# GuixingLin/akka-allreduce

Hardware: AMD Instinct MI355X
Metric: allreduce algbw (GB/s) on 256 MB fp32 buffer at 1/2/4/8 MI355X (higher is better)
Workload: dtype fp32

## Files before the change

### akka_allreduce_amd/models/mlp.py

```python
from __future__ import annotations

from typing import Optional

import torch
import torch.nn as nn
import torch.nn.functional as F

from ..ops.colsum import colsum
from ..ops.xent import cross_entropy
from ..parallel.dp import AllreduceFn, GradientBucket


def _mm_into(a: torch.Tensor, b: torch.Tensor, out: torch.Tensor) -> None:
    if a.dtype == out.dtype:
        torch.mm(a, b, out=out)
        return
    try:
        torch.mm(a, b, out_dtype=out.dtype, out=out)
    except (TypeError, RuntimeError):
        out.copy_(torch.mm(a, b))


class _LinearIntoBucket(torch.autograd.Function):

    @staticmethod
    def forward(ctx, x, w, b, gw, gb, ws=None, bs=None):
        dt = torch.get_autocast_dtype(x.device.type) if torch.is_autocast_enabled(x.device.type) else None
        with torch.autocast(device_type=x.device.type, enabled=False):
            if dt is not None and ws is not None and bs is not None and ws.dtype == dt and bs.dtype == dt:
                xc, wc, bc = x.to(dt), ws, bs
            elif dt is not None:
                xc, wc, bc = x.to(dt), w.to(dt), b.to(dt)
            else:
                xc, wc, bc = x, w, b
            y = F.linear(xc, wc, bc)
        ctx.save_for_backward(xc, wc)
        ctx.gw, ctx.gb = gw, gb
        return y

    @staticmethod
    def backward(ctx, go):
        xc, wc = ctx.saved_tensors
        go2 = go.reshape(-1, go.shape[-1]).to(wc.dtype)
        _mm_into(go2.t(), xc.reshape(-1, xc.shape[-1]), ctx.gw)
        if go2.is_cuda and go2.dtype == torch.bfloat16 and ctx.gb.dtype == torch.float32 and ctx.gb.is_contiguous():
            colsum(go2, out=ctx.gb.view(-1))
        else:
            torch.sum(go2, 0, dtype=ctx.gb.dtype, out=ctx.gb)
        gx = (go2 @ wc).reshape(*go.shape[:-1], wc.shape[1]) if ctx.needs_input_grad[0] else None
        return gx, None, None, None, None, None, None


class _LinearReluIntoBucket(torch.autograd.Function):

    @staticmethod
    def forward(ctx, x, w, b, gw, gb, ws, bs):
        dt = torch.get_autocast_dtype(x.device.type)
        with torch.autocast(device_type=x.device.type, enabled=False):
            xc = x.to(dt)
            wc = ws if ws is not None else w.to(dt)
            bc = bs if bs is not None else b.to(dt)
            x2 = xc.reshape(-1, xc.shape[-1])
            h = torch._addmm_activation(bc, x2, wc.t(), use_gelu=False)
        ctx.save_for_backward(x2, wc, h)
        ctx.gw, ctx.gb, ctx.xshape = gw, gb, xc.shape
        return h.reshape(*xc.shape[:-1], wc.shape[0])

    @staticmethod
    def backward(ctx, go):
        x2, wc, h = ctx.saved_tensors
        go2 = go.reshape(-1, go.shape[-1]).to(wc.dtype).contiguous()
        g = torch.empty_like(go2)
        colsum(go2, out=ctx.gb.view(-1), relu_of=h, masked_out=g)
        _mm_into(g.t(), x2, ctx.gw)
        gx = (g @ wc).reshape(ctx.xshape) if ctx.needs_input_grad[0] else None
        return gx, None, None, None, None, None, None


class MLP(nn.Module):
    def __init__(self, d_in: int, d_hidden: int, d_out: int):
        super().__init__()
        self.fc1 = nn.Linear(d_in, d_hidden)
        self.fc2 = nn.Linear(d_hidden, d_out)
        self.direct_grads = False
        self.last_step_direct = False
        self.shadow_bucket: Optional[GradientBucket] = None

    def _linear(self, fc: nn.Linear, x: torch.Tensor) -> torch.Tensor:
        if self.direct_grads and torch.is_grad_enabled():
            sb = self.shadow_bucket
            ws = sb.shadow_of(fc.weight) if sb is not None else None
            bs = sb.shadow_of(fc.bias) if sb is not None else None
            return _LinearIntoBucket.apply(x, fc.weight, fc.bias, fc.weight.grad, fc.bias.grad, ws, bs)
        return fc(x)

    def _linear_relu(self, fc: nn.Linear, x: torch.Tensor) -> torch.Tensor:
        if (self.direct_grads and torch.is_grad_enabled() and x.is_cuda and torch.is_autocast_enabled("cuda")
                and torch.get_autocast_dtype("cuda") == torch.bfloat16 and fc.bias is not None
                and fc.bias.grad is not None and fc.bias.grad.is_contiguous()):
            sb = self.shadow_bucket
            ws = sb.shadow_of(fc.weight) if sb is not None else None
            bs = sb.shadow_of(fc.bias) if sb is not None else None
            return _LinearReluIntoBucket.apply(x, fc.weight, fc.bias, fc.weight.grad, fc.bias.grad, ws, bs)
        return F.relu(self._linear(fc, x))

    def forward(self, x: torch.Tensor) -> torch.Tensor:
        return self._linear(self.fc2, self._linear_relu(self.fc1, x))


def dp_sgd_step(model: nn.Module, x: torch.Tensor, y: torch.Tensor, lr: float,
                allreduce: Optional[AllreduceFn], bucket: Optional[GradientBucket] = None,
                sync_loss: bool = True, compute_dtype: Optional[torch.dtype] = None,
                direct_grads: bool = True, shadow_weights: bool = True, fused_loss: bool = True,
                optimizer=None):
    if optimizer is not None:
        if bucket is not None and optimizer.bucket is not bucket:
            raise ValueError("dp_sgd_step: the optimizer was built on another bucket")
        bucket = optimizer.bucket
    if bucket is None:
        bucket = getattr(model, "_akka_bucket", None)
        if bucket is None:
            bucket = GradientBucket(list(model.parameters()))
            model._akka_bucket = bucket
    loss = _forward_backward(model, x, y, bucket, compute_dtype, direct_grads, shadow_weights, fused_loss)
    bucket.update_from(allreduce, lr, optimizer or bucket.sgd)
    return float(loss.detach()) if sync_loss else loss.detach()


def _forward_backward(model: nn.Module, x: torch.Tensor, y: torch.Tensor, bucket: GradientBucket,
                      compute_dtype: Optional[torch.dtype], direct_grads: bool, shadow_weights: bool,
                      fused_loss: bool, grad_seed: Optional[torch.Tensor] = None) -> torch.Tensor:
    bucket.rebind()
    direct = isinstance(model, MLP) and direct_grads and bucket.bound() \
        and set(map(id, model.parameters())) == set(map(id, bucket.params))
    try:
        if direct:
            model.direct_grads = True
            lowp = compute_dtype if (shadow_weights and compute_dtype is not None
                                     and compute_dtype != torch.float32) else None
            model.shadow_bucket = bucket if bucket.use_shadow(lowp) else None
        else:
            bucket.use_shadow(None)
            bucket.zero_()
        if compute_dtype is not None and compute_dtype != torch.float32:
            with torch.autocast(device_type=x.device.type, dtype=compute_dtype):
                logits = model(x)
            loss = cross_entropy(logits, y) if fused_loss else F.cross_entropy(logits.float(), y)
        else:
            loss = F.cross_entropy(model(x), y)
        loss.backward(grad_seed)
    finally:
        if isinstance(model, MLP):
            model.direct_grads = False
            model.shadow_bucket = None
            model.last_step_direct = direct
    return loss


class GraphedDPStep:

    def __init__(self, model: "MLP", bucket: GradientBucket, x: torch.Tensor, y: torch.Tensor,
                 compute_dtype: Optional[torch.dtype] = None, shadow_weights: bool = True, warmup: int = 3,
                 allreduce: Optional[AllreduceFn] = None, lr: Optional[float] = None, optimizer=None):
        if not (x.is_cuda and isinstance(model, MLP)):
            raise ValueError("GraphedDPStep: an MLP on a GPU")
        if optimizer is not None and optimizer.bucket is not bucket:
            raise ValueError("GraphedDPStep: the optimizer was built on another bucket")
        if bucket.pflat is None or not bucket.bound() or not bucket.params_bound():
            raise ValueError("GraphedDPStep: needs GradientBucket(flatten_params=True) bound to the model")
        self.model, self.bucket, self.rule = model, bucket, optimizer or bucket.sgd
        self.compute_dtype = compute_dtype
        self.lowp = compute_dtype if (shadow_weights and compute_dtype is not None
                                      and compute_dtype != torch.float32) else None
        lowx = compute_dtype if (compute_dtype is not None and compute_dtype != torch.float32
                                 and x.is_floating_point() and x.dtype == torch.float32) else None
        self.sx = x.detach().to(lowx) if lowx is not None else x.detach().clone()
        self.sy = y.detach().clone()
        self._seed = torch.ones((), dtype=torch.float32, device=x.device)
        self._ptrs = self._pointers()

        self.allreduce = allreduce if (allreduce is not None and getattr(allreduce, "capturable", False)) else None
        if allreduce is not None and self.allreduce is None:
            raise ValueError("GraphedDPStep: this allreduce keeps host-side round state; pass it at call time")
        if self.allreduce is not None and lr is None:
            raise ValueError("GraphedDPStep: a captured update needs its learning rate")
        self.lr = lr
        self._out = torch.empty_like(bucket.wire if bucket.wire is not None else bucket.flat) \
            if self.allreduce is not None else None
        self.replays = 0

        def fb():
            loss = _forward_backward(model, self.sx, self.sy, bucket, compute_dtype, True, shadow_weights, True,
                                     grad_seed=self._seed)
            if self.allreduce is not None:
                bucket.update_from(self.allreduce, float(lr), self.rule, out_buf=self._out)
            return loss

        side = torch.cuda.Stream(device=x.device)
        side.wait_stream(torch.cuda.current_stream(x.device))
        snap = (bucket.snapshot(), [s.clone() for s in self.rule.state_tensors()]) \
            if self.allreduce is not None else None
        with torch.cuda.stream(side):
            for _ in range(warmup):
                fb()
        side.synchronize()
        self._side = side
        self.graph = torch.cuda.CUDAGraph()
        with torch.cuda.graph(self.graph, stream=side):
            self.loss = fb().detach()
        torch.cuda.current_stream(x.device).wait_stream(side)
        if snap is not None:
            bucket.restore(snap[0])
            for s, keep in zip(self.rule.state_tensors(), snap[1]):
                s.copy_(keep)
            if self._device_lr():
                self.rule.set_lr(float(lr))
        self._ptrs = self._pointers()

    def static_inputs(self):
        return self.sx, self.sy

    def _pointers(self):
        return self.bucket.pointers(), self.rule.state_pointers()

    def _device_lr(self) -> bool:
        return bool(getattr(self.rule, "device_lr", False))

    def __call__(self, x: torch.Tensor, y: torch.Tensor, lr: float, allreduce: Optional[AllreduceFn],
                 sync_loss: bool = False):
        b = self.bucket
        if self._pointers() != self._ptrs:
            raise RuntimeError("GraphedDPStep: a parameter, gradient, shadow, wire, residual or optimizer state "
                               "buffer moved since the capture")
        if b.use_shadow(self.lowp) != (self.lowp is not None and b.sflat is not None):
            raise RuntimeError("GraphedDPStep: the bf16 shadow is no longer usable")
        if x.data_ptr() != self.sx.data_ptr():
            self.sx.copy_(x)
        if y.data_ptr() != self.sy.data_ptr():
            self.sy.copy_(y)
        if self.allreduce is not None:
            if allreduce is not None and allreduce is not self.allreduce:
                raise RuntimeError("GraphedDPStep: the step captured another allreduce")
            if self._device_lr():
                if lr != self.rule.lr:
                    self.rule.set_lr(lr)
                self.lr = lr
            elif lr != self.lr:
                raise RuntimeError(f"GraphedDPStep: the update was captured with lr={self.lr}")
            self.graph.replay()
            self.replays += 1
            self.allreduce.note_replays(1)
            b.shadow_written()
        else:
            self.graph.replay()
            b.update_from(allreduce, lr, self.rule)
        return float(self.loss) if sync_loss else self.loss


def synthetic_batch(batch: int, d_in: int, n_classes: int, *, device, generator: Optional[torch.Generator] = None):
    x = torch.randn(batch, d_in, device=device, generator=generator)
    w = torch.arange(d_in * n_classes, device=device, dtype=torch.float32).reshape(d_in, n_classes).sin()
    y = (x @ w).argmax(dim=1)
    return x, y
```

### akka_allreduce_amd/ops/__init__.py

```python
from .colsum import colsum
from .compress import pack_bf16
from .reduce import chunk_reduce, count_expand
from .xent import cross_entropy

__all__ = ["chunk_reduce", "colsum", "count_expand", "cross_entropy", "pack_bf16"]
```

### akka_allreduce_amd/ops/xent.py

```python
from __future__ import annotations

import os
from typing import Dict, Tuple

import torch
import torch.nn.functional as F

from .._native_loader import load as _load

_TICKETS: Dict[Tuple[int, int], torch.Tensor] = {}
_CHECK_LABELS = os.environ.get("AKKA_CHECK_LABELS") == "1"
_LAST: Dict[int, torch.Tensor] = {}


def last_bad_labels() -> int:
    out = _LAST.get(0)
    return int(out[2].item()) if out is not None else 0


def _ticket(dev: torch.device, stream: int) -> torch.Tensor:
    key = (dev.index or 0, stream)
    t = _TICKETS.get(key)
    if t is None:
        t = torch.zeros(1, dtype=torch.int32, device=dev)
        _TICKETS[key] = t
    return t


class _FusedXent(torch.autograd.Function):
    @staticmethod
    def forward(ctx, logits: torch.Tensor, target: torch.Tensor):
        x = logits.contiguous()
        y = target.contiguous().to(torch.int64)
        B, C = x.shape
        stream = torch.cuda.current_stream(x.device).cuda_stream
        lse = torch.empty(B, dtype=torch.float32, device=x.device)
        rowloss = torch.empty(2 * B, dtype=torch.float32, device=x.device)
        out = torch.empty(3, dtype=torch.float32, device=x.device)
        _load().xent_fwd(x.data_ptr(), y.data_ptr(), B, C, lse.data_ptr(), rowloss.data_ptr(), out.data_ptr(),
                         _ticket(x.device, stream).data_ptr(), stream)
        ctx.save_for_backward(x, y, lse, out)
        if _CHECK_LABELS and float(out[2].item()) > 0:
            raise ValueError(f"cross_entropy: {int(out[2].item())} target(s) outside [0, {C}) "
                             "(only -100 is ignored)")
        _LAST[0] = out
        return out[0]

    @staticmethod
    def backward(ctx, go: torch.Tensor):
        x, y, lse, out = ctx.saved_tensors
        B, C = x.shape
        g = go.to(torch.float32).contiguous()
        gx = torch.empty_like(x)
        _load().xent_bwd(x.data_ptr(), y.data_ptr(), B, C, lse.data_ptr(), out.data_ptr(), g.data_ptr(),
                         gx.data_ptr(), torch.cuda.current_stream(x.device).cuda_stream)
        return gx, None


def cross_entropy(logits: torch.Tensor, target: torch.Tensor) -> torch.Tensor:
    if (logits.is_cuda and logits.dtype == torch.bfloat16 and logits.dim() == 2 and target.dim() == 1
            and target.shape[0] == logits.shape[0] and logits.shape[0] > 0):
        return _FusedXent.apply(logits, target)
    return F.cross_entropy(logits, target)
```

### csrc/bindings/bindings.cpp

```cpp
#include <hip/hip_runtime.h>
#include <pybind11/functional.h>
#include <pybind11/pybind11.h>
#include <pybind11/stl.h>

#include <algorithm>
#include <chrono>
#include <condition_variable>
#include <cstdlib>
#include <cstring>
#include <deque>
#include <map>
#include <mutex>
#include <set>

#include "../engine/engine.h"
#include "../kernels/kernels.h"
#include "../runtime/frames.h"
#include "../runtime/watchdog.h"
#include "../transport/ipc_p2p.h"
#include "../transport/p2p.h"
#include "../transport/reactive_link.h"
#include "harness_p2p.h"
#include "../transport/stream_link.h"

// ... 880 lines not shown
    for (int32_t t = 0; t < tournament_rounds(n); ++t) {
      std::vector<int32_t> partner(static_cast<size_t>(n), 0);
      for (int32_t x = 0; x < n; ++x) partner[size_t(x)] = tournament_partner(n, t, x);
      rounds.push_back(partner);
    }
    return rounds;
  }, "partner[x] per ncclCommSplit round of the pair-communicator setup (>= n: sits out)");

  py::class_<P2P>(m, "P2PEndpoint")
      .def("rank", &P2P::rank)
      .def("nranks", &P2P::nranks)
      .def("info", [](const P2P& p) {
        P2PInfo i = p.info();
        py::dict d;
        d["kind"] = i.kind;
        d["nranks"] = i.nranks;
        d["rank"] = i.rank;
        d["device"] = i.device;
        d["comms"] = i.comms;
        return d;
      })
      .def("check", &P2P::check)
      .def("has_collectives", &P2P::has_collectives)
      .def("rebuild", [](P2P& p, py::bytes uid, std::vector<int32_t> members) {
        std::string s = uid;
        return p.rebuild(std::vector<uint8_t>(s.begin(), s.end()), members);
      })
      .def("reduce_scatter", [](P2P& p, uintptr_t stream, uintptr_t send, uintptr_t recv, size_t count,
                                const std::string& dtype) {
        p.reduce_scatter(reinterpret_cast<StreamH>(stream), reinterpret_cast<const void*>(send),
                         reinterpret_cast<void*>(recv), count, dtype == "bfloat16" ? DType::BF16 : DType::F32);
      })
      .def("all_gather", [](P2P& p, uintptr_t stream, uintptr_t send, uintptr_t recv, size_t count,
                            const std::string& dtype) {
        p.all_gather(reinterpret_cast<StreamH>(stream), reinterpret_cast<const void*>(send),
                     reinterpret_cast<void*>(recv), count, dtype == "bfloat16" ? DType::BF16 : DType::F32);
      })
      .def("group", [](P2P& p, uintptr_t stream, const std::vector<std::tuple<bool, int32_t, uintptr_t, size_t>>& ops) {
        std::vector<P2POp> v;
        v.reserve(ops.size());
        for (const auto& o : ops)
          v.push_back({std::get<0>(o), std::get<1>(o), reinterpret_cast<void*>(std::get<2>(o)), std::get<3>(o)});
        p.group(reinterpret_cast<StreamH>(stream), v);
      });
  m.def("rccl_endpoint", [](py::bytes uid, int32_t rank, int32_t nranks, int32_t device, bool pairs,
                            std::vector<int32_t> members) {
    std::string s = uid;
    std::vector<uint8_t> v(s.begin(), s.end());
    return pairs ? make_rccl_pair_p2p(v, rank, nranks, device) : make_rccl_p2p(v, rank, nranks, device, members);
  }, py::arg("uid"), py::arg("rank"), py::arg("nranks"), py::arg("device"), py::arg("pairs") = false,
     py::arg("members") = std::vector<int32_t>{});

  m.def("reduce", [](uintptr_t dst, std::vector<uintptr_t> srcs, int64_t n, std::string dtype, uintptr_t stream,
                     std::string impl) {
    const DType dt = parse_dtype(dtype);
    ReduceImpl im = reduce_impl_from_name(impl.c_str());
    std::vector<const void*> ptrs;
    for (auto p : srcs) ptrs.push_back(reinterpret_cast<const void*>(p));
    AKKA_CHECK(!ptrs.empty(), "reduce: no sources");
    for (const auto& spec : split_reduce(reinterpret_cast<void*>(dst), ptrs, n)) launch_reduce(as_stream(stream), spec, dt, im);
  }, py::arg("dst"), py::arg("srcs"), py::arg("n"), py::arg("dtype") = "float32", py::arg("stream") = 0,
        py::arg("impl") = "auto");
  m.def("count_expand", [](uintptr_t out, const CountsArgs& table, uintptr_t stream) {
    launch_count_expand(as_stream(stream), reinterpret_cast<int32_t*>(out), counts_table(table));
  });
  m.def("count_mean", [](uintptr_t dst, uintptr_t src, const CountsArgs& table, const std::string& dtype,
                         uintptr_t stream, bool axpy, float alpha, uintptr_t shadow, const std::string& src_dtype) {
    const DType dt = parse_dtype(dtype);
    launch_count_mean(as_stream(stream), reinterpret_cast<void*>(dst), reinterpret_cast<const void*>(src),
                      counts_table(table), dt, src_dtype.empty() ? dt : parse_dtype(src_dtype), axpy, alpha,
                      reinterpret_cast<void*>(shadow));
  }, py::arg("dst"), py::arg("src"), py::arg("table"), py::arg("dtype"), py::arg("stream"), py::arg("axpy") = false,
     py::arg("alpha") = 0.f, py::arg("shadow") = 0, py::arg("src_dtype") = "");
  m.def("count_optim", [](const std::string& kind, uintptr_t p, uintptr_t mom, uintptr_t v, uintptr_t shadow,
                          uintptr_t src, const std::string& src_dtype, const CountsArgs& table, uintptr_t t,
                          uintptr_t sq, uintptr_t stream, bool nt, double lr, double weight_decay, double momentum,
                          bool nesterov, double beta1, double beta2, double eps, double max_norm,
                          const std::string& state_dtype, uint32_t seed) {
    AKKA_CHECK(kind == "sgd" || kind == "adamw", "count_optim: kind is 'sgd' or 'adamw'");
    const OptimSpec o{kind == "adamw" ? OptimKind::AdamW : OptimKind::SGD, lr, weight_decay, momentum, nesterov,
                      beta1, beta2, eps, max_norm};
    launch_count_optim(as_stream(stream), reinterpret_cast<float*>(p), reinterpret_cast<void*>(mom),
                       reinterpret_cast<void*>(v), parse_dtype(state_dtype), reinterpret_cast<void*>(shadow),
                       reinterpret_cast<const void*>(src), parse_dtype(src_dtype), counts_table(table), o,
                       reinterpret_cast<const int32_t*>(t), reinterpret_cast<const float*>(sq), seed, nt);
  }, py::arg("kind"), py::arg("p"), py::arg("m"), py::arg("v"), py::arg("shadow"), py::arg("src"),
     py::arg("src_dtype"), py::arg("table"), py::arg("t"), py::arg("sq"), py::arg("stream") = 0,
     py::arg("nt") = false, py::kw_only(), py::arg("lr"), py::arg("weight_decay") = 0.0, py::arg("momentum") = 0.0,
     py::arg("nesterov") = false, py::arg("beta1") = 0.9, py::arg("beta2") = 0.999, py::arg("eps") = 1e-8,
     py::arg("max_norm") = 0.0, py::arg("state_dtype") = "float32", py::arg("seed") = 0u);
  m.def("count_optim_groups", [](const std::string& kind, uintptr_t p, uintptr_t mom, uintptr_t v, uintptr_t shadow,
                                 uintptr_t src, const std::string& src_dtype, const CountsArgs& table, uintptr_t t,
                                 uintptr_t sq, uintptr_t seg_end, uintptr_t seg_group, uintptr_t rows,
                                 const std::vector<int64_t>& host_seg_end, const std::vector<int32_t>& host_seg_group,
                                 int32_t ngroups, uintptr_t stream, double momentum, bool nesterov, double beta1,
                                 double beta2, double eps, double max_norm, const std::string& state_dtype,
                                 uint32_t seed) {
    AKKA_CHECK(kind == "sgd" || kind == "adamw", "count_optim_groups: kind is 'sgd' or 'adamw'");
    AKKA_CHECK(!host_seg_end.empty() && host_seg_end.size() == host_seg_group.size(),
               "count_optim_groups: one group per segment");
    const OptimSpec o{kind == "adamw" ? OptimKind::AdamW : OptimKind::SGD, 0.0, 0.0, momentum, nesterov,
                      beta1, beta2, eps, max_norm};
    OptimGroups g;
    g.seg_end = reinterpret_cast<const int64_t*>(seg_end);
    g.seg_group = reinterpret_cast<const int32_t*>(seg_group);
    g.rows = reinterpret_cast<const float*>(rows);
    g.nseg = int32_t(host_seg_end.size());
    g.ngroups = ngroups;
    g.host_seg_end = host_seg_end.data();
    g.host_seg_group = host_seg_group.data();
    launch_count_optim_groups(as_stream(stream), reinterpret_cast<float*>(p), reinterpret_cast<void*>(mom),
                              reinterpret_cast<void*>(v), parse_dtype(state_dtype), reinterpret_cast<void*>(shadow),
                              reinterpret_cast<const void*>(src), parse_dtype(src_dtype), counts_table(table), o, g,
                              reinterpret_cast<const int32_t*>(t), reinterpret_cast<const float*>(sq), seed);
  }, py::arg("kind"), py::arg("p"), py::arg("m"), py::arg("v"), py::arg("shadow"), py::arg("src"),
     py::arg("src_dtype"), py::arg("table"), py::arg("t"), py::arg("sq"), py::arg("seg_end"), py::arg("seg_group"),
     py::arg("rows"), py::arg("host_seg_end"), py::arg("host_seg_group"), py::arg("ngroups"), py::arg("stream") = 0,
     py::kw_only(), py::arg("momentum") = 0.0, py::arg("nesterov") = false, py::arg("beta1") = 0.9,
     py::arg("beta2") = 0.999, py::arg("eps") = 1e-8, py::arg("max_norm") = 0.0,
     py::arg("state_dtype") = "float32", py::arg("seed") = 0u);
  m.def("count_sqnorm", [](uintptr_t sq, uintptr_t src, const std::string& src_dtype, const CountsArgs& table,
                           uintptr_t part, uintptr_t ticket, uintptr_t stream) {
    launch_count_sqnorm(as_stream(stream), reinterpret_cast<float*>(sq), reinterpret_cast<const void*>(src),
                        parse_dtype(src_dtype), counts_table(table), reinterpret_cast<float*>(part),
                        reinterpret_cast<uint32_t*>(ticket));
  }, py::arg("sq"), py::arg("src"), py::arg("src_dtype"), py::arg("table"), py::arg("part"), py::arg("ticket"),
     py::arg("stream") = 0);
  m.def("count_sqnorm_partials", &count_sqnorm_partials);
  m.def("pack_bf16", [](uintptr_t dst, uintptr_t src, uintptr_t residual, int64_t n, uintptr_t stream) {
    AKKA_CHECK(n >= 0 && (n == 0 || (dst != 0 && src != 0)), "pack_bf16: null buffer");
    launch_pack_bf16(as_stream(stream), reinterpret_cast<void*>(dst), reinterpret_cast<const float*>(src),
                     reinterpret_cast<float*>(residual), n);
  }, py::arg("dst"), py::arg("src"), py::arg("residual"), py::arg("n"), py::arg("stream") = 0);
  m.def("colsum_bf16", [](uintptr_t out, uintptr_t in, int64_t M, int64_t ncol, uintptr_t part, uintptr_t tickets,
                          int32_t splits, uintptr_t stream, bool lite, uintptr_t act, uintptr_t gout) {
    launch_colsum_bf16(as_stream(stream), reinterpret_cast<float*>(out), reinterpret_cast<const void*>(in), M, ncol,
                       reinterpret_cast<float*>(part), reinterpret_cast<uint32_t*>(tickets), splits, lite,
                       reinterpret_cast<const void*>(act), reinterpret_cast<void*>(gout));
  }, py::arg("out"), py::arg("in"), py::arg("M"), py::arg("ncol"), py::arg("part"), py::arg("tickets"),
     py::arg("splits"), py::arg("stream"), py::arg("lite") = true, py::arg("act") = 0, py::arg("gout") = 0);
  m.def("colsum_row_splits", &colsum_row_splits);
  m.def("xent_fwd", [](uintptr_t x, uintptr_t y, int64_t B, int64_t C, uintptr_t lse, uintptr_t rowloss, uintptr_t out,
                       uintptr_t ticket, uintptr_t stream) {
    launch_xent_fwd(as_stream(stream), reinterpret_cast<const void*>(x), reinterpret_cast<const int64_t*>(y), B, C,
                    reinterpret_cast<float*>(lse), reinterpret_cast<float*>(rowloss), reinterpret_cast<float*>(out),
                    reinterpret_cast<uint32_t*>(ticket));
  });
  m.def("xent_bwd", [](uintptr_t x, uintptr_t y, int64_t B, int64_t C, uintptr_t lse, uintptr_t stat, uintptr_t go,
                       uintptr_t gx, uintptr_t stream) {
    launch_xent_bwd(as_stream(stream), reinterpret_cast<const void*>(x), reinterpret_cast<const int64_t*>(y), B, C,
                    reinterpret_cast<const float*>(lse), reinterpret_cast<const float*>(stat),
                    reinterpret_cast<const float*>(go), reinterpret_cast<void*>(gx));
  });
  m.def("geometry", [](int64_t S, int32_t N, int64_t C) {
    Geometry g(S, N, C);
    py::dict d;
    std::vector<std::pair<int64_t, int64_t>> blocks;
    std::vector<int32_t> nch;
    for (int32_t j = 0; j < N; ++j) {
      blocks.push_back({g.block_start(j), g.block_end(j)});
      nch.push_back(g.num_chunks(j));
    }
    d["step"] = g.step;
    d["blocks"] = blocks;
    d["num_chunks"] = nch;
    d["total_chunks"] = g.total_chunks();
    return d;
  });
  m.def("float_threshold", &float_threshold);
  m.def("ipc_p2p_plan", [](std::vector<std::tuple<bool, int32_t, int64_t, int32_t>> ops, int32_t nranks,
                           int64_t piece, std::vector<uint32_t> dead, std::vector<uint32_t> send_seq,
                           std::vector<uint32_t> recv_seq) {
    std::vector<P2POp> v;
    for (auto& t : ops) v.push_back({std::get<0>(t), std::get<1>(t), nullptr, size_t(std::get<2>(t)), std::get<3>(t)});
    dead.resize(size_t(nranks), 0);
    IpcP2PPlan plan = plan_ipc_p2p_group(v, nranks, piece, 2, dead.data(), send_seq, recv_seq);
    py::list queues;
    for (size_t q = 0; q + 1 < plan.qstart.size(); ++q) {
      py::list ql;
      for (int32_t i = plan.qstart[q]; i < plan.qstart[q + 1]; ++i) {
        const IpcP2POp& o = plan.ops[size_t(i)];
        ql.append(py::make_tuple(bool(o.send), int(o.peer), int(o.ch), o.bytes, o.seq));
      }
      queues.append(ql);
    }
    return py::make_tuple(queues, send_seq, recv_seq, plan.bytes_sent);
  });
  m.def("ipc_layout", [](int32_t N, int32_t np, int32_t nslots, int32_t wpp) {
    py::dict d;
    std::vector<int64_t> lane, p2p;
    for (int32_t src = 0; src < N; ++src)
      for (int32_t j = 0; j < np; ++j) lane.push_back(ipc_flag_push(src, j, np));
    for (int32_t j = 0; j < np; ++j)
      for (int32_t part = 0; part < kIpcReduceSplit; ++part) lane.push_back(ipc_flag_reduced(j, part, N, np));
    for (int32_t src = 0; src < N; ++src)
      for (int32_t j = 0; j < np; ++j)
        for (int32_t part = 0; part < kIpcReduceSplit; ++part) lane.push_back(ipc_flag_gather(src, j, part, N, np));
    lane.push_back(ipc_flag_error(N, np));
    for (int32_t r = 0; r < N; ++r)
      for (int32_t ch = 0; ch < 2; ++ch)
        for (int32_t sl = 0; sl < nslots; ++sl)
          for (int32_t w = 0; w < wpp; ++w) {
            p2p.push_back(ipc_p2p_flag_written(r, ch, sl, w, 2, nslots, wpp));
            p2p.push_back(ipc_p2p_flag_consumed(r, ch, sl, w, N, 2, nslots, wpp));
          }
    d["lane_flags"] = lane;
    d["lane_flag_bytes"] = int64_t(ipc_flag_bytes(N, np));
    d["p2p_flags"] = p2p;
    d["p2p_flag_bytes"] = int64_t(ipc_p2p_flag_bytes(N, 2, nslots, wpp));
    d["stride"] = kIpcFlagStride;
    d["window_slots"] = ipc_window_slots(N);
    return d;
  });
  m.attr("build_arch") = "gfx950";
}
```

### csrc/kernels/kernels.h

```cpp
#pragma once

#include <hip/hip_runtime.h>

#include "../engine/device.h"

namespace akka {

enum class ReduceImpl : int32_t {
  Auto = 0,
  Vec = 1,
  Lds = 2,
  Scalar = 3,
  VecNts = 4,
  VecNtl = 5,
  VecBoth = 6,
};
ReduceImpl reduce_impl_from_name(const char* name);

void launch_reduce(hipStream_t s, const ReduceSpec& spec, DType dt, ReduceImpl impl);
struct CountsTable {
  const int32_t* counts;
  int64_t S, step;
  int32_t N;
  int64_t C;
  int32_t kmax;
  int64_t regions() const { return int64_t(N) * kmax; }
  void check(const char* who) const {
    AKKA_CHECK(regions() > 0 && step >= 0 && C > 0, std::string(who) + ": bad geometry");
  }
};
void launch_count_expand(hipStream_t s, int32_t* out, const CountsTable& t);
void launch_count_mean(hipStream_t s, void* dst, const void* src, const CountsTable& t, DType dt, DType src_dt,
                       bool axpy = false, float alpha = 0.f, void* shadow = nullptr);
enum class OptimKind : int32_t { SGD = 0, AdamW = 1 };
struct OptimSpec {
  OptimKind kind = OptimKind::SGD;
  double lr = 0, weight_decay = 0;
  double momentum = 0;
  bool nesterov = false;
  double beta1 = 0.9, beta2 = 0.999, eps = 1e-8;
  double max_norm = 0;
};
void launch_count_optim(hipStream_t s, float* p, void* m, void* v, DType state_dt, void* shadow, const void* src,
                        DType src_dt, const CountsTable& ct, const OptimSpec& o, const int32_t* t, const float* sq,
                        uint32_t seed = 0, bool nt = false);
struct OptimGroups {
  const int64_t* seg_end = nullptr;
  const int32_t* seg_group = nullptr;
  const float* rows = nullptr;
  int32_t nseg = 0, ngroups = 0;
  const int64_t* host_seg_end = nullptr;
  const int32_t* host_seg_group = nullptr;
};
void launch_count_optim_groups(hipStream_t s, float* p, void* m, void* v, DType state_dt, void* shadow,
                               const void* src, DType src_dt, const CountsTable& ct, const OptimSpec& o,
                               const OptimGroups& g, const int32_t* t, const float* sq, uint32_t seed = 0);
void launch_count_sqnorm(hipStream_t s, float* sq, const void* src, DType src_dt, const CountsTable& ct, float* part,
                         uint32_t* ticket);
int32_t count_sqnorm_partials();
void launch_pack_bf16(hipStream_t s, void* q, const float* g, float* r, int64_t n);
void launch_colsum_bf16(hipStream_t s, float* out, const void* in, int64_t M, int64_t ncol, float* part,
                        uint32_t* tickets, int32_t splits, bool lite = true, const void* act = nullptr,
                        void* gout = nullptr);
int32_t colsum_row_splits(int64_t M, int64_t ncol);
void launch_xent_fwd(hipStream_t s, const void* x, const int64_t* y, int64_t B, int64_t C, float* lse,
                     float* rowloss, float* out, uint32_t* ticket);
void launch_xent_bwd(hipStream_t s, const void* x, const int64_t* y, int64_t B, int64_t C, const float* lse,
                     const float* stat, const float* go, void* gx);
void launch_poison_counts(hipStream_t s, const uint32_t* flag, int32_t* counts, int64_t n);
void launch_fill_counts(hipStream_t s, const uint32_t* flag, int32_t* counts, int32_t value, int64_t n);
ReduceImpl reduce_impl_from_env();
const char* reduce_impl_name(ReduceImpl i);

}
```

### csrc/kernels/xent.hip

```cpp
#include <hip/hip_runtime.h>

#include "elem.h"
#include "kernels.h"
#include "launch_util.h"
#include "xgmi_device.h"

namespace akka {

namespace {

using Bf16 = Elt<bf16_t>;

__device__ __forceinline__ float block_reduce(float v, float* red, bool is_max) {
  for (int o = 32; o > 0; o >>= 1) {
    const float w = __shfl_xor(v, o, 64);
    v = is_max ? fmaxf(v, w) : v + w;
  }
  __syncthreads();
  if ((threadIdx.x & 63) == 0) red[threadIdx.x >> 6] = v;
  __syncthreads();
  float r = red[0];
  for (int w = 1; w < int(blockDim.x >> 6); ++w) r = is_max ? fmaxf(r, red[w]) : r + red[w];
  return r;
}

constexpr int64_t kIgnoreIndex = -100;

__global__ __launch_bounds__(kBlock) void xent_fwd_kernel(const bf16_t* __restrict__ x, const int64_t* __restrict__ y,
                                                          int64_t B, int64_t C, float* __restrict__ lse,
                                                          float* __restrict__ rowloss, float* __restrict__ out,
                                                          uint32_t* __restrict__ ticket) {
  __shared__ float red[kBlock / 64 + 1];
  const int64_t r = blockIdx.x;
  const bf16_t* row = x + r * C;
  float m = -INFINITY;
  for (int64_t c = threadIdx.x; c < C; c += kBlock) m = fmaxf(m, Bf16::to_f(row[c]));
  m = block_reduce(m, red, true);
  float sum = 0.f;
  for (int64_t c = threadIdx.x; c < C; c += kBlock) sum += __expf(Bf16::to_f(row[c]) - m);
  sum = block_reduce(sum, red, false);
  const auto rs = xgmi::sys_rsrc(rowloss, B * 8);
  if (threadIdx.x == 0) {
    const float l = m + __logf(sum);
    const int64_t t = y[r];
    const bool valid = t >= 0 && t < C;
    const float flag = valid ? 1.f : (t == kIgnoreIndex ? 0.f : -1.f);
    lse[r] = l;
    __builtin_amdgcn_raw_buffer_store_b32(__float_as_uint(valid ? l - Bf16::to_f(row[t]) : 0.f), rs, int(r * 8), 0,
                                          xgmi::kSysAux);
    __builtin_amdgcn_raw_buffer_store_b32(__float_as_uint(flag), rs, int(r * 8 + 4), 0, xgmi::kSysAux);
    asm volatile("s_waitcnt vmcnt(0)" ::: "memory");
    red[kBlock / 64] =
        __hip_atomic_fetch_add(ticket, 1u, __ATOMIC_RELAXED, __HIP_MEMORY_SCOPE_AGENT) == uint32_t(B - 1) ? 1.f : 0.f;
  }
  __syncthreads();
  if (red[kBlock / 64] == 0.f) return;
  float ls = 0.f, nv = 0.f, nb = 0.f;
  for (int64_t i = threadIdx.x; i < B; i += kBlock) {
    ls += __uint_as_float(__builtin_amdgcn_raw_buffer_load_b32(rs, int(i * 8), 0, xgmi::kSysAux));
    const float f = __uint_as_float(__builtin_amdgcn_raw_buffer_load_b32(rs, int(i * 8 + 4), 0, xgmi::kSysAux));
    nv += f > 0.f ? f : 0.f;
    nb += f < 0.f ? 1.f : 0.f;
  }
  ls = block_reduce(ls, red, false);
  nv = block_reduce(nv, red, false);
  nb = block_reduce(nb, red, false);
  if (threadIdx.x == 0) {
    out[0] = (nv > 0.f && nb == 0.f) ? ls / nv : __uint_as_float(0x7fc00000u);
    out[1] = nv;
    out[2] = nb;
    __hip_atomic_store(ticket, 0u, __ATOMIC_RELAXED, __HIP_MEMORY_SCOPE_AGENT);
  }
}

__global__ __launch_bounds__(kBlock) void xent_bwd_kernel(const bf16_t* __restrict__ x, const int64_t* __restrict__ y,
                                                          int64_t C, const float* __restrict__ lse,
                                                          const float* __restrict__ stat,
                                                          const float* __restrict__ go, bf16_t* __restrict__ gx) {
  const int64_t r = blockIdx.x;
  const int64_t t = y[r];
  const float nv = stat[1];
  const float scale = (t >= 0 && t < C && nv > 0.f && stat[2] == 0.f) ? go[0] / nv : 0.f;
  const float l = lse[r];
  const bf16_t* row = x + r * C;
  bf16_t* g = gx + r * C;
  for (int64_t c = threadIdx.x; c < C; c += kBlock) {
    const float p = __expf(Bf16::to_f(row[c]) - l) - (c == t ? 1.f : 0.f);
    g[c] = Bf16::from_f(p * scale);
  }
}

}

void launch_xent_fwd(hipStream_t s, const void* x, const int64_t* y, int64_t B, int64_t C, float* lse,
                     float* rowloss, float* out, uint32_t* ticket) {
  AKKA_CHECK(B >= 1 && C >= 1 && B < (int64_t(1) << 27), "xent: bad shape");
  hipLaunchKernelGGL(xent_fwd_kernel, dim3(uint32_t(B)), dim3(kBlock), 0, s, static_cast<const bf16_t*>(x), y, B, C,
                     lse, rowloss, out, ticket);
  check_launch("xent_fwd");
}

void launch_xent_bwd(hipStream_t s, const void* x, const int64_t* y, int64_t B, int64_t C, const float* lse,
                     const float* stat, const float* go, void* gx) {
  AKKA_CHECK(B >= 1 && C >= 1, "xent: bad shape");
  hipLaunchKernelGGL(xent_bwd_kernel, dim3(uint32_t(B)), dim3(kBlock), 0, s, static_cast<const bf16_t*>(x), y, C, lse,
                     stat, go, static_cast<bf16_t*>(gx));
  check_launch("xent_bwd");
}

}
```

Before: 3554.

## Fuse cross-entropy forward, backward and fc2 bias-gradient sum into one head kernel

```diff
diff --git a/akka_allreduce_amd/models/mlp.py b/akka_allreduce_amd/models/mlp.py
--- a/akka_allreduce_amd/models/mlp.py
+++ b/akka_allreduce_amd/models/mlp.py
@@ -7,7 +7,7 @@
 import torch.nn.functional as F
 
 from ..ops.colsum import colsum
-from ..ops.xent import cross_entropy
+from ..ops.xent import cross_entropy, cross_entropy_head, head_rows, unit_seed
 from ..parallel.dp import AllreduceFn, GradientBucket
 
 
@@ -43,7 +43,9 @@
         xc, wc = ctx.saved_tensors
         go2 = go.reshape(-1, go.shape[-1]).to(wc.dtype)
         _mm_into(go2.t(), xc.reshape(-1, xc.shape[-1]), ctx.gw)
-        if go2.is_cuda and go2.dtype == torch.bfloat16 and ctx.gb.dtype == torch.float32 and ctx.gb.is_contiguous():
+        if ctx.gb is None:
+            pass
+        elif go2.is_cuda and go2.dtype == torch.bfloat16 and ctx.gb.dtype == torch.float32 and ctx.gb.is_contiguous():
             colsum(go2, out=ctx.gb.view(-1))
         else:
             torch.sum(go2, 0, dtype=ctx.gb.dtype, out=ctx.gb)
@@ -85,13 +87,15 @@
         self.direct_grads = False
         self.last_step_direct = False
         self.shadow_bucket: Optional[GradientBucket] = None
+        self.head_sums_fc2_bias = False
 
     def _linear(self, fc: nn.Linear, x: torch.Tensor) -> torch.Tensor:
         if self.direct_grads and torch.is_grad_enabled():
             sb = self.shadow_bucket
             ws = sb.shadow_of(fc.weight) if sb is not None else None
             bs = sb.shadow_of(fc.bias) if sb is not None else None
-            return _LinearIntoBucket.apply(x, fc.weight, fc.bias, fc.weight.grad, fc.bias.grad, ws, bs)
+            gb = None if (fc is self.fc2 and self.head_sums_fc2_bias) else fc.bias.grad
+            return _LinearIntoBucket.apply(x, fc.weight, fc.bias, fc.weight.grad, gb, ws, bs)
         return fc(x)
 
     def _linear_relu(self, fc: nn.Linear, x: torch.Tensor) -> torch.Tensor:
@@ -112,7 +116,7 @@
                 allreduce: Optional[AllreduceFn], bucket: Optional[GradientBucket] = None,
                 sync_loss: bool = True, compute_dtype: Optional[torch.dtype] = None,
                 direct_grads: bool = True, shadow_weights: bool = True, fused_loss: bool = True,
-                optimizer=None):
+                optimizer=None, fused_head: bool = True):
     if optimizer is not None:
         if bucket is not None and optimizer.bucket is not bucket:
             raise ValueError("dp_sgd_step: the optimizer was built on another bucket")
@@ -122,14 +126,16 @@
         if bucket is None:
             bucket = GradientBucket(list(model.parameters()))
             model._akka_bucket = bucket
-    loss = _forward_backward(model, x, y, bucket, compute_dtype, direct_grads, shadow_weights, fused_loss)
+    loss = _forward_backward(model, x, y, bucket, compute_dtype, direct_grads, shadow_weights, fused_loss,
+                             fused_head=fused_head)
     bucket.update_from(allreduce, lr, optimizer or bucket.sgd)
     return float(loss.detach()) if sync_loss else loss.detach()
 
 
 def _forward_backward(model: nn.Module, x: torch.Tensor, y: torch.Tensor, bucket: GradientBucket,
                       compute_dtype: Optional[torch.dtype], direct_grads: bool, shadow_weights: bool,
-                      fused_loss: bool, grad_seed: Optional[torch.Tensor] = None) -> torch.Tensor:
+                      fused_loss: bool, grad_seed: Optional[torch.Tensor] = None,
+                      fused_head: bool = True) -> torch.Tensor:
     bucket.rebind()
     direct = isinstance(model, MLP) and direct_grads and bucket.bound() \
         and set(map(id, model.parameters())) == set(map(id, bucket.params))
@@ -142,10 +148,26 @@
         else:
             bucket.use_shadow(None)
             bucket.zero_()
+        db2 = model.fc2.bias.grad if direct and model.fc2.bias is not None else None
+        head = (direct and fused_head and fused_loss and compute_dtype == torch.bfloat16 and x.is_cuda
+                and x.dim() == 2 and y.dim() == 1 and y.shape[0] == x.shape[0]
+                and head_rows(x.shape[0], model.fc2.out_features) > 0
+                and db2 is not None and db2.dtype == torch.float32 and db2.is_contiguous()
+                and (grad_seed is None or (grad_seed.is_cuda and grad_seed.dtype == torch.float32
+                                           and grad_seed.numel() == 1)))
         if compute_dtype is not None and compute_dtype != torch.float32:
+            if head:
+                model.head_sums_fc2_bias = True
             with torch.autocast(device_type=x.device.type, dtype=compute_dtype):
                 logits = model(x)
-            loss = cross_entropy(logits, y) if fused_loss else F.cross_entropy(logits.float(), y)
+            if head:
+                if logits.dtype != torch.bfloat16 or logits.shape != (x.shape[0], model.fc2.out_features):
+                    raise RuntimeError("dp_sgd_step: the loss head does not take these logits")
+                if grad_seed is None:
+                    grad_seed = unit_seed(logits.device)
+                loss = cross_entropy_head(logits, y, grad_seed, db2.view(-1))
+            else:
+                loss = cross_entropy(logits, y) if fused_loss else F.cross_entropy(logits.float(), y)
         else:
             loss = F.cross_entropy(model(x), y)
         loss.backward(grad_seed)
@@ -153,6 +175,7 @@
         if isinstance(model, MLP):
             model.direct_grads = False
             model.shadow_bucket = None
+            model.head_sums_fc2_bias = False
             model.last_step_direct = direct
     return loss
 
diff --git a/akka_allreduce_amd/ops/__init__.py b/akka_allreduce_amd/ops/__init__.py
--- a/akka_allreduce_amd/ops/__init__.py
+++ b/akka_allreduce_amd/ops/__init__.py
@@ -1,6 +1,6 @@
 from .colsum import colsum
 from .compress import pack_bf16
 from .reduce import chunk_reduce, count_expand
-from .xent import cross_entropy
+from .xent import cross_entropy, cross_entropy_head
 
-__all__ = ["chunk_reduce", "colsum", "count_expand", "cross_entropy", "pack_bf16"]
+__all__ = ["chunk_reduce", "colsum", "count_expand", "cross_entropy", "cross_entropy_head", "pack_bf16"]
diff --git a/akka_allreduce_amd/ops/xent.py b/akka_allreduce_amd/ops/xent.py
--- a/akka_allreduce_amd/ops/xent.py
+++ b/akka_allreduce_amd/ops/xent.py
@@ -1,7 +1,7 @@
 from __future__ import annotations
 
 import os
-from typing import Dict, Tuple
+from typing import Dict, Optional, Tuple
 
 import torch
 import torch.nn.functional as F
@@ -57,6 +57,108 @@
         return gx, None
 
 
+_HEAD_WS: Dict[Tuple[int, int, int, int, int], Tuple[torch.Tensor, torch.Tensor]] = {}
+_ONES: Dict[int, torch.Tensor] = {}
+
+
+def unit_seed(dev: torch.device) -> torch.Tensor:
+    key = dev.index or 0
+    t = _ONES.get(key)
+    if t is None:
+        t = torch.ones((), dtype=torch.float32, device=dev)
+        _ONES[key] = t
+    return t
+
+
+def head_rows(B: int, C: int) -> int:
+    return int(_load().xent_head_rows(int(B), int(C)))
+
+
+def _check_db(db_out: torch.Tensor, logits: torch.Tensor) -> None:
+    if (db_out.dtype != torch.float32 or db_out.numel() != logits.shape[1] or not db_out.is_contiguous()
+            or db_out.device != logits.device):
+        raise ValueError("cross_entropy_head: db_out must be a contiguous fp32 tensor of logits.shape[1] elements "
+                         "on the logits' device")
+
+
+class _XentHead(torch.autograd.Function):
+
+    @staticmethod
+    def forward(ctx, logits: torch.Tensor, target: torch.Tensor, seed: torch.Tensor, db_out: torch.Tensor,
+                rows: int):
+        x = logits.contiguous()
+        y = target.contiguous().to(torch.int64)
+        B, C = x.shape
+        dev = x.device
+        stream = torch.cuda.current_stream(dev).cuda_stream
+        key = (dev.index or 0, stream, B, C, rows)
+        ws = _HEAD_WS.get(key)
+        if ws is None:
+            ws = (torch.empty(2 * B, dtype=torch.float32, device=dev),
+                  torch.empty(((B + rows - 1) // rows, C), dtype=torch.float32, device=dev))
+            _HEAD_WS[key] = ws
+        lse = torch.empty(B, dtype=torch.float32, device=dev)
+        out = torch.empty(3, dtype=torch.float32, device=dev)
+        gx = torch.empty_like(x)
+        _load().xent_head(x.data_ptr(), y.data_ptr(), B, C, seed.data_ptr(), lse.data_ptr(), ws[0].data_ptr(),
+                          ws[1].data_ptr(), out.data_ptr(), gx.data_ptr(), db_out.data_ptr(),
+                          _ticket(dev, stream).data_ptr(), rows, stream)
+        ctx.save_for_backward(x, y, lse, out, gx)
+        ctx.seed, ctx.seed_version, ctx.db_out = seed, seed._version, db_out
+        if _CHECK_LABELS and float(out[2].item()) > 0:
+            raise ValueError(f"cross_entropy: {int(out[2].item())} target(s) outside [0, {C}) "
+                             "(only -100 is ignored)")
+        _LAST[0] = out
+        return out[0]
+
+    @staticmethod
+    def backward(ctx, go: torch.Tensor):
+        x, y, lse, out, gx = ctx.saved_tensors
+        seed = ctx.seed
+        if (go.dtype == torch.float32 and go.numel() == 1 and go.device == seed.device
+                and go.data_ptr() == seed.data_ptr() and seed._version == ctx.seed_version):
+            return gx, None, None, None, None
+        from .colsum import colsum
+
+        B, C = x.shape
+        g = go.to(torch.float32).contiguous()
+        gx = torch.empty_like(x)
+        _load().xent_bwd(x.data_ptr(), y.data_ptr(), B, C, lse.data_ptr(), out.data_ptr(), g.data_ptr(),
+                         gx.data_ptr(), torch.cuda.current_stream(x.device).cuda_stream)
+        colsum(gx, out=ctx.db_out.view(-1))
+        return gx, None, None, None, None
+
+
+class _XentTwoKernels(torch.autograd.Function):
+
+    @staticmethod
+    def forward(ctx, logits: torch.Tensor, target: torch.Tensor, db_out: torch.Tensor):
+        ctx.db_out = db_out
+        return _FusedXent.forward(ctx, logits, target)
+
+    @staticmethod
+    def backward(ctx, go: torch.Tensor):
+        from .colsum import colsum
+
+        gx, _ = _FusedXent.backward(ctx, go)
+        colsum(gx, out=ctx.db_out.view(-1))
+        return gx, None, None
+
+
+def cross_entropy_head(logits: torch.Tensor, target: torch.Tensor, seed: torch.Tensor, db_out: torch.Tensor,
+                       rows: Optional[int] = None) -> torch.Tensor:
+    if not (logits.is_cuda and logits.dtype == torch.bfloat16 and logits.dim() == 2 and target.dim() == 1
+            and target.shape[0] == logits.shape[0] and logits.shape[0] > 0 and logits.shape[1] > 0):
+        raise ValueError("cross_entropy_head: CUDA bf16 logits [B, C] and targets [B]")
+    if not (seed.is_cuda and seed.device == logits.device and seed.dtype == torch.float32 and seed.numel() == 1):
+        raise ValueError("cross_entropy_head: the seed is one fp32 element on the logits' device")
+    _check_db(db_out, logits)
+    default = head_rows(*logits.shape)
+    if default == 0:
+        return _XentTwoKernels.apply(logits, target, db_out)
+    return _XentHead.apply(logits, target, seed, db_out, int(rows or default))
+
+
 def cross_entropy(logits: torch.Tensor, target: torch.Tensor) -> torch.Tensor:
     if (logits.is_cuda and logits.dtype == torch.bfloat16 and logits.dim() == 2 and target.dim() == 1
             and target.shape[0] == logits.shape[0] and logits.shape[0] > 0):
diff --git a/csrc/bindings/bindings.cpp b/csrc/bindings/bindings.cpp
--- a/csrc/bindings/bindings.cpp
+++ b/csrc/bindings/bindings.cpp
@@ -1056,6 +1056,16 @@
                     reinterpret_cast<const float*>(lse), reinterpret_cast<const float*>(stat),
                     reinterpret_cast<const float*>(go), reinterpret_cast<void*>(gx));
   });
+  m.def("xent_head", [](uintptr_t x, uintptr_t y, int64_t B, int64_t C, uintptr_t go, uintptr_t lse,
+                        uintptr_t rowloss, uintptr_t part, uintptr_t out, uintptr_t gx, uintptr_t db,
+                        uintptr_t ticket, int32_t rows_per_wg, uintptr_t stream) {
+    launch_xent_head(as_stream(stream), reinterpret_cast<const void*>(x), reinterpret_cast<const int64_t*>(y), B, C,
+                     reinterpret_cast<const float*>(go), reinterpret_cast<float*>(lse),
+                     reinterpret_cast<float*>(rowloss), reinterpret_cast<float*>(part), reinterpret_cast<float*>(out),
+                     reinterpret_cast<void*>(gx), reinterpret_cast<float*>(db), reinterpret_cast<uint32_t*>(ticket),
+                     rows_per_wg);
+  });
+  m.def("xent_head_rows", &xent_head_rows);
   m.def("geometry", [](int64_t S, int32_t N, int64_t C) {
     Geometry g(S, N, C);
     py::dict d;
diff --git a/csrc/kernels/kernels.h b/csrc/kernels/kernels.h
--- a/csrc/kernels/kernels.h
+++ b/csrc/kernels/kernels.h
@@ -67,6 +67,10 @@
                      float* rowloss, float* out, uint32_t* ticket);
 void launch_xent_bwd(hipStream_t s, const void* x, const int64_t* y, int64_t B, int64_t C, const float* lse,
                      const float* stat, const float* go, void* gx);
+void launch_xent_head(hipStream_t s, const void* x, const int64_t* y, int64_t B, int64_t C, const float* go,
+                      float* lse, float* rowloss, float* part, float* out, void* gx, float* db, uint32_t* ticket,
+                      int32_t rows_per_wg);
+int32_t xent_head_rows(int64_t B, int64_t C);
 void launch_poison_counts(hipStream_t s, const uint32_t* flag, int32_t* counts, int64_t n);
 void launch_fill_counts(hipStream_t s, const uint32_t* flag, int32_t* counts, int32_t value, int64_t n);
 ReduceImpl reduce_impl_from_env();
diff --git a/csrc/kernels/xent.hip b/csrc/kernels/xent.hip
--- a/csrc/kernels/xent.hip
+++ b/csrc/kernels/xent.hip
@@ -11,11 +11,16 @@
 
 using Bf16 = Elt<bf16_t>;
 
-__device__ __forceinline__ float block_reduce(float v, float* red, bool is_max) {
+__device__ __forceinline__ float wave_reduce(float v, bool is_max) {
   for (int o = 32; o > 0; o >>= 1) {
     const float w = __shfl_xor(v, o, 64);
     v = is_max ? fmaxf(v, w) : v + w;
   }
+  return v;
+}
+
+__device__ __forceinline__ float block_reduce(float v, float* red, bool is_max) {
+  v = wave_reduce(v, is_max);
   __syncthreads();
   if ((threadIdx.x & 63) == 0) red[threadIdx.x >> 6] = v;
   __syncthreads();
@@ -90,6 +95,264 @@
   }
 }
 
+constexpr int kHeadWaves = 8;
+constexpr int kHeadBlock = 64 * kHeadWaves;
+constexpr int kHeadMaxB = 4096;
+constexpr int kHeadMaxGroups = 64;
+constexpr int kHeadMaxVpl = 2;
+constexpr int kHeadLabels = 4;
+constexpr int kHeadCombine = 32;
+constexpr uint32_t kNegInf2 = 0xff80ff80u;
+
+template <bool MAX, int CTRL, int ROWS>
+__device__ __forceinline__ float dpp_step(float v) {
+  const float id = MAX ? -INFINITY : 0.f;
+  const float w =
+      __int_as_float(__builtin_amdgcn_update_dpp(__float_as_int(id), __float_as_int(v), CTRL, ROWS, 0xf, false));
+  return MAX ? fmaxf(v, w) : v + w;
+}
+template <bool MAX>
+__device__ __forceinline__ float wave_reduce_dpp(float v) {
+  v = dpp_step<MAX, 0xb1, 0xf>(v);
+  v = dpp_step<MAX, 0x4e, 0xf>(v);
+  v = dpp_step<MAX, 0x141, 0xf>(v);
+  v = dpp_step<MAX, 0x140, 0xf>(v);
+  v = dpp_step<MAX, 0x142, 0xa>(v);
+  v = dpp_step<MAX, 0x143, 0xc>(v);
+  return __int_as_float(__builtin_amdgcn_readlane(__float_as_int(v), 63));
+}
+
+template <bool VEC>
+__device__ __forceinline__ void head_combine(__amdgpu_buffer_rsrc_t rs, __amdgpu_buffer_rsrc_t prs, int64_t B,
+                                             int64_t C, int groups, float* __restrict__ out, float* __restrict__ db,
+                                             float (*red)[kHeadWaves], uint32_t* __restrict__ ticket) {
+  const uint32_t l0 = __builtin_amdgcn_raw_buffer_load_b32(rs, int(threadIdx.x * 8), 0, xgmi::kSysAux);
+  const uint32_t f0 = __builtin_amdgcn_raw_buffer_load_b32(rs, int(threadIdx.x * 8 + 4), 0, xgmi::kSysAux);
+  constexpr int W = VEC ? 2 : 1;
+  for (int64_t c = int64_t(threadIdx.x) * W; c < C; c += kHeadBlock * W) {
+    float s[W];
+#pragma unroll
+    for (int e = 0; e < W; ++e) s[e] = 0.f;
+    for (int g0 = 0; g0 < groups; g0 += kHeadCombine) {
+      uint32_t v[kHeadCombine][W];
+#pragma unroll
+      for (int u = 0; u < kHeadCombine; ++u) {
+        const int off = int((int64_t(g0 + u) * C + c) * 4);
+        if constexpr (VEC) {
+          const auto w = __builtin_amdgcn_raw_buffer_load_b64(prs, off, 0, xgmi::kSysAux);
+          v[u][0] = w[0];
+          v[u][1] = w[1];
+        } else {
+          v[u][0] = __builtin_amdgcn_raw_buffer_load_b32(prs, off, 0, xgmi::kSysAux);
+        }
+      }
+#pragma unroll
+      for (int u = 0; u < kHeadCombine; ++u)
+#pragma unroll
+        for (int e = 0; e < W; ++e) s[e] += __uint_as_float(v[u][e]);
+    }
+#pragma unroll
+    for (int e = 0; e < W; ++e) db[c + e] = s[e];
+  }
+  float ls = 0.f, nv = 0.f, nb = 0.f;
+  auto add_row = [&](uint32_t lw, uint32_t fw) {
+    const float f = __uint_as_float(fw);
+    ls += __uint_as_float(lw);
+    nv += f > 0.f ? f : 0.f;
+    nb += f < 0.f ? 1.f : 0.f;
+  };
+  add_row(l0, f0);
+  for (int64_t i = int64_t(threadIdx.x) + kHeadBlock; i < B; i += kHeadBlock)
+    add_row(__builtin_amdgcn_raw_buffer_load_b32(rs, int(i * 8), 0, xgmi::kSysAux),
+            __builtin_amdgcn_raw_buffer_load_b32(rs, int(i * 8 + 4), 0, xgmi::kSysAux));
+  ls = wave_reduce_dpp<false>(ls);
+  nv = wave_reduce_dpp<false>(nv);
+  nb = wave_reduce_dpp<false>(nb);
+  if ((threadIdx.x & 63) == 0) {
+    red[0][threadIdx.x >> 6] = ls;
+    red[1][threadIdx.x >> 6] = nv;
+    red[2][threadIdx.x >> 6] = nb;
+  }
+  __syncthreads();
+  if (threadIdx.x == 0) {
+    ls = red[0][0], nv = red[1][0], nb = red[2][0];
+    for (int w = 1; w < kHeadWaves; ++w) ls += red[0][w], nv += red[1][w], nb += red[2][w];
+    out[0] = (nv > 0.f && nb == 0.f) ? ls / nv : __uint_as_float(0x7fc00000u);
+    out[1] = nv;
+    out[2] = nb;
+    __hip_atomic_store(ticket, 0u, __ATOMIC_RELAXED, __HIP_MEMORY_SCOPE_AGENT);
+  }
+}
+
+template <int VPL>
+__global__ __launch_bounds__(kHeadBlock) void xent_head_kernel(const bf16_t* __restrict__ x,
+                                                           const int64_t* __restrict__ y, int64_t B, int64_t C,
+                                                           int32_t rows_per_wg, const float* __restrict__ go,
+                                                           float* __restrict__ lse, float* __restrict__ rowloss,
+                                                           float* __restrict__ part, float* __restrict__ out,
+                                                           bf16_t* gx, float* __restrict__ db,
+                                                           uint32_t* __restrict__ ticket) {
+  constexpr int kStage = VPL > 0 ? VPL * 64 * 9 : 1;
+  __shared__ float stage[kHeadWaves][kStage];
+  __shared__ float red[3][kHeadWaves];
+  __shared__ uint32_t last;
+  const int lane = threadIdx.x & 63, wave = threadIdx.x >> 6;
+  auto scale_of_batch = [&]() {
+    int nv = 0, nb = 0;
+    for (int64_t w0 = 0; w0 < B; w0 += 64 * kHeadLabels) {
+      const int64_t i0 = w0 + lane;
+      int64_t t[kHeadLabels];
+#pragma unroll
+      for (int u = 0; u < kHeadLabels; ++u) t[u] = y[i0 + 64 * u < B ? i0 + 64 * u : B - 1];
+#pragma unroll
+      for (int u = 0; u < kHeadLabels; ++u) {
+        const bool in = i0 + 64 * u < B, valid = t[u] >= 0 && t[u] < C;
+        nv += __popcll(__ballot(in && valid));
+        nb += __popcll(__ballot(in && !valid && t[u] != kIgnoreIndex));
+      }
+    }
+    return (nv > 0 && nb == 0) ? go[0] / float(nv) : 0.f;
+  };
+
+  const int64_t r0 = int64_t(blockIdx.x) * rows_per_wg;
+  const int64_t r1 = r0 + rows_per_wg < B ? r0 + rows_per_wg : B;
+  const auto rs = xgmi::sys_rsrc(rowloss, B * 8);
+  const auto prs = xgmi::sys_rsrc(part, int64_t(gridDim.x) * C * 4);
+  auto put_row = [&](int64_t r, float loss, int64_t t, bool valid) {
+    const float flag = valid ? 1.f : (t == kIgnoreIndex ? 0.f : -1.f);
+    __builtin_amdgcn_raw_buffer_store_b32(__float_as_uint(loss), rs, int(r * 8), 0, xgmi::kSysAux);
+    __builtin_amdgcn_raw_buffer_store_b32(__float_as_uint(flag), rs, int(r * 8 + 4), 0, xgmi::kSysAux);
+  };
+
+  if constexpr (VPL > 0) {
+    float acc[VPL][8];
+#pragma unroll
+    for (int j = 0; j < VPL; ++j)
+#pragma unroll
+      for (int q = 0; q < 8; ++q) acc[j][q] = 0.f;
+    auto load_row = [&](int64_t r, v4u (&v)[VPL]) {
+#pragma unroll
+      for (int j = 0; j < VPL; ++j) {
+        const int64_t c = int64_t(lane + 64 * j) * 8;
+        v[j] = c < C ? *reinterpret_cast<const v4u*>(x + r * C + c) : v4u{kNegInf2, kNegInf2, kNegInf2, kNegInf2};
+      }
+    };
+    v4u cur[VPL], nxt[VPL];
+#pragma unroll
+    for (int j = 0; j < VPL; ++j) nxt[j] = v4u{0u, 0u, 0u, 0u};
+    int64_t t = 0, tn = 0;
+    int64_t r = r0 + wave;
+    if (r < r1) {
+      load_row(r, cur);
+      t = y[r];
+    }
+    const float scale_valid = scale_of_batch();
+    for (; r < r1; r += kHeadWaves) {
+      if (r + kHeadWaves < r1) {
+        load_row(r + kHeadWaves, nxt);
+        tn = y[r + kHeadWaves];
+      }
+      float f[VPL][8];
+      float m = -INFINITY;
+#pragma unroll
+      for (int j = 0; j < VPL; ++j)
+#pragma unroll
+        for (int q = 0; q < 8; ++q) {
+          f[j][q] = unit_elem<bf16_t>(&cur[j], q);
+          m = fmaxf(m, f[j][q]);
+        }
+      m = wave_reduce_dpp<true>(m);
+      float sum = 0.f;
+#pragma unroll
+      for (int j = 0; j < VPL; ++j)
+#pragma unroll
+        for (int q = 0; q < 8; ++q) sum += __expf(f[j][q] - m);
+      sum = wave_reduce_dpp<false>(sum);
+      const float l = m + __logf(sum);
+      const bool valid = t >= 0 && t < C;
+      const float scale = valid ? scale_valid : 0.f;
+      bool mine = false;
+      float xt = 0.f;
+#pragma unroll
+      for (int j = 0; j < VPL; ++j) {
+        const int64_t c = int64_t(lane + 64 * j) * 8;
+        float g[8];
+#pragma unroll
+        for (int q = 0; q < 8; ++q) {
+          const bool hit = c + q == t;
+          if (hit) {
+            mine = true;
+            xt = f[j][q];
+          }
+          g[q] = (__expf(f[j][q] - l) - (hit ? 1.f : 0.f)) * scale;
+        }
+        if (c < C) {
+          const v4u p = Bf16::pack(g);
+          *reinterpret_cast<v4u*>(gx + r * C + c) = p;
+          Bf16::add(acc[j], p);
+        }
+      }
+      if (lane == 0) lse[r] = l;
+      if (valid ? mine : lane == 0) put_row(r, valid ? l - xt : 0.f, t, valid);
+#pragma unroll
+      for (int j = 0; j < VPL; ++j) cur[j] = nxt[j];
+      t = tn;
+    }
+#pragma unroll
+    for (int j = 0; j < VPL; ++j)
+#pragma unroll
+      for (int q = 0; q < 8; ++q) stage[wave][(lane + 64 * j) * 9 + q] = acc[j][q];
+    __syncthreads();
+    for (int64_t c = int64_t(threadIdx.x) * 4; c < C; c += kHeadBlock * 4) {
+      const int li = int(c + (c >> 3));
+      v4u p;
+#pragma unroll
+      for (int e = 0; e < 4; ++e)
+      {
+        float sum = stage[0][li + e];
+#pragma unroll
+        for (int w = 1; w < kHeadWaves; ++w) sum += stage[w][li + e];
+        p[e] = __float_as_uint(sum);
+      }
+      __builtin_amdgcn_raw_buffer_store_b128(p, prs, int((int64_t(blockIdx.x) * C + c) * 4), 0, xgmi::kSysAux);
+    }
+  } else {
+    const float scale_valid = scale_of_batch();
+    for (int64_t r = r0 + wave; r < r1; r += kHeadWaves) {
+      const bf16_t* row = x + r * C;
+      const int64_t t = y[r];
+      const bool valid = t >= 0 && t < C;
+      float m = -INFINITY;
+      for (int64_t c = lane; c < C; c += 64) m = fmaxf(m, Bf16::to_f(row[c]));
+      m = wave_reduce_dpp<true>(m);
+      float sum = 0.f;
+      for (int64_t c = lane; c < C; c += 64) sum += __expf(Bf16::to_f(row[c]) - m);
+      sum = wave_reduce_dpp<false>(sum);
+      const float l = m + __logf(sum);
+      const float scale = valid ? scale_valid : 0.f;
+      for (int64_t c = lane; c < C; c += 64)
+        gx[r * C + c] = Bf16::from_f((__expf(Bf16::to_f(row[c]) - l) - (c == t ? 1.f : 0.f)) * scale);
+      if (lane == 0) {
+        lse[r] = l;
+        put_row(r, valid ? l - Bf16::to_f(row[t]) : 0.f, t, valid);
+      }
+    }
+    xgmi::drain_wg();
+    for (int64_t c = threadIdx.x; c < C; c += kHeadBlock) {
+      float s = 0.f;
+      for (int64_t r = r0; r < r1; ++r) s += Bf16::to_f(gx[r * C + c]);
+      __builtin_amdgcn_raw_buffer_store_b32(__float_as_uint(s), prs, int((int64_t(blockIdx.x) * C + c) * 4), 0,
+                                            xgmi::kSysAux);
+    }
+  }
+  xgmi::drain_wg();
+  if (threadIdx.x == 0)
+    last = __hip_atomic_fetch_add(ticket, 1u, __ATOMIC_RELAXED, __HIP_MEMORY_SCOPE_AGENT) == gridDim.x - 1 ? 1u : 0u;
+  __syncthreads();
+  if (!last) return;
+  head_combine<(VPL > 0)>(rs, prs, B, C, int(gridDim.x), out, db, red, ticket);
+}
+
 }
 
 void launch_xent_fwd(hipStream_t s, const void* x, const int64_t* y, int64_t B, int64_t C, float* lse,
@@ -108,4 +371,29 @@
   check_launch("xent_bwd");
 }
 
-}
+int32_t xent_head_rows(int64_t B, int64_t C) {
+  if (B < 1 || B > kHeadMaxB || C < 1) return 0;
+  const int64_t per_wave = (B + int64_t(kHeadWaves) * kHeadMaxGroups - 1) / (int64_t(kHeadWaves) * kHeadMaxGroups);
+  return int32_t(per_wave * kHeadWaves);
+}
+
+void launch_xent_head(hipStream_t s, const void* x, const int64_t* y, int64_t B, int64_t C, const float* go,
+                      float* lse, float* rowloss, float* part, float* out, void* gx, float* db, uint32_t* ticket,
+                      int32_t rows_per_wg) {
+  AKKA_CHECK(B >= 1 && B <= kHeadMaxB && C >= 1, "xent_head: bad shape (1 <= B <= 4096)");
+  AKKA_CHECK(rows_per_wg >= 1, "xent_head: bad rows per workgroup");
+  const int64_t groups = (B + rows_per_wg - 1) / rows_per_wg;
+  AKKA_CHECK(groups * C * 4 < (int64_t(1) << 31), "xent_head: partial rows exceed 2 GiB");
+  const bool vec = ((reinterpret_cast<uintptr_t>(x) | reinterpret_cast<uintptr_t>(gx)) & 15) == 0 && C % 8 == 0 &&
+                   C <= 64 * 8 * kHeadMaxVpl;
+  const int vpl = !vec ? 0 : C <= 512 ? 1 : kHeadMaxVpl;
+  const bool ok = dispatch_int<0, 1, kHeadMaxVpl>(vpl, [&](auto V) {
+    hipLaunchKernelGGL((xent_head_kernel<decltype(V)::value>), dim3(uint32_t(groups)), dim3(kHeadBlock), 0, s,
+                       static_cast<const bf16_t*>(x), y, B, C, rows_per_wg, go, lse, rowloss, part, out,
+                       static_cast<bf16_t*>(gx), db, ticket);
+  });
+  AKKA_CHECK(ok, "xent_head: no kernel for this row width");
+  check_launch("xent_head");
+}
+
+}
```

Measured after the change: 3524. Within noise of the previous version (-0.8%).
